# DonghuiZhuo/kube-batch-1

Measured on AMD Instinct MI355X. Metric: pod placements/sec + p50 session latency, 100k nodes × 1M pods, higher is better.
Workload: dtype int64

## Files before the change

kube-batch-1_amd/csrc/engine/engine_dev.h:

```cpp
#pragma once
#include <hip/hip_runtime.h>

#define KBHIP_STAMPS_OFF
#include "../kbhip_batch.h"
#include "../kbhip_engine.h"

namespace kbhip {

constexpr uint64_t kEngWaitTicks = 200000000ull;
constexpr uint64_t kEngArriveTicks = 500000ull;
constexpr uint64_t kEngDescTicks = 400000000ull;

__device__ __forceinline__ uint64_t eng_now() { return __builtin_amdgcn_s_memrealtime(); }

#define ETL(A, p, ev)                                                                                    \
    do {                                                                                                 \
        if ((A).tl && (threadIdx.x & 63) == 0)                                                           \
            (A).tl[(size_t)((p) % kEngTlSlots) * kEngTlEvents + (ev)] = __builtin_amdgcn_s_memrealtime(); \
    } while (0)

#ifndef KBHIP_POLL_DEPTH
#define KBHIP_POLL_DEPTH 1
#endif
#ifndef KBHIP_POLL_SLEEP
// ... 33 lines not shown
__device__ __forceinline__ T eng_uniform(const T& v) {
    static_assert(sizeof(T) % 4 == 0, "dwords");
    T r;
    const uint32_t* s = (const uint32_t*)&v;
    uint32_t* d = (uint32_t*)&r;
#pragma unroll
    for (int i = 0; i < (int)(sizeof(T) / 4); ++i) d[i] = (uint32_t)__builtin_amdgcn_readfirstlane((int)s[i]);
    return r;
}

__device__ __forceinline__ TaskClass eng_class(const uint32_t* w) {
    return eng_uniform(*(const TaskClass*)(w + kEngDescClass));
}
__device__ __forceinline__ TaskClass eng_class_x(uint32_t x) {
    TaskClass c;
    uint32_t* d = (uint32_t*)&c;
#pragma unroll
    for (int i = 0; i < (int)(sizeof(TaskClass) / 4); ++i)
        d[i] = (uint32_t)__builtin_amdgcn_readlane((int)x, kEngDescClass + i);
    return c;
}

struct EngDesc {
    uint32_t op, cls, m, gang, ent32, min_avail, ready, epoch, slot;
    int32_t kbase, kshift, kidxmax;
};
__device__ __forceinline__ EngDesc eng_decode(const uint32_t* w) {
    EngDesc d;
    d.cls = w[kDwCls];
    d.m = w[kDwFlags] & 0xff;
    d.gang = (w[kDwFlags] >> 8) & 1;
    d.ent32 = (w[kDwFlags] >> 9) & 1;
    d.op = (w[kDwFlags] >> 12) & 0xf;
    d.min_avail = w[kDwMinAvail];
    d.ready = w[kDwReady];
    d.epoch = w[kDwEpochSlot] & 0xffff;
    d.slot = w[kDwEpochSlot] >> 16;
    d.kbase = (int32_t)w[kDwKbase];
    d.kshift = (int32_t)w[kDwKshift];
    d.kidxmax = (int32_t)w[kDwKidxmax];
    return d;
}
__device__ __forceinline__ PopArgs eng_args(const EngDesc& d) {
    PopArgs a{};
    a.cls = (int32_t)d.cls;
    a.n_tasks = (int32_t)d.m;
    a.gang_mode = (int32_t)d.gang;
    a.min_avail = (int32_t)d.min_avail;
    a.ready_count = (int32_t)d.ready;
    a.epoch = d.epoch;
    a.placement = 2;
    a.kbase = d.kbase;
    a.kshift = d.kshift;
    a.kidxmax = d.kidxmax;
    a.ent32 = (int32_t)d.ent32;
    a.fit_set = 0;
    return a;
}

__device__ __forceinline__ bool eng_wait_desc(EngCtl* ctl, uint32_t p, uint32_t* w) {
    const int lane = threadIdx.x & 63;
    const uint64_t* src = &ctl->desc[p % kEngRing][lane];
    EngWait wt(ctl, kEngDescTicks);
    for (;;) {
        const uint64_t x = ld_sc1(src);
        if (__ballot((uint32_t)(x >> 32) != p) == 0) {
            w[lane] = (uint32_t)x;
            return true;
        }
        if (!wt.tick(kEngErrDesc)) return false;
    }
}

__device__ __forceinline__ bool eng_wait_done(EngCtl* ctl, uint32_t want) {
    EngWait wt(ctl, kEngWaitTicks);
    for (;;) {
        const uint32_t v = (uint32_t)__builtin_amdgcn_readfirstlane((int)ld_sc1(&ctl->done));
        if ((int32_t)(v - want) >= 0) return true;
        if (!wt.tick()) return false;
    }
}

constexpr int kPollDepth = KBHIP_POLL_DEPTH;
__device__ __forceinline__ bool eng_poll_tag(EngCtl* ctl, const uint64_t* w, uint32_t q, uint64_t limit) {
    uint64_t v[kPollDepth];
#pragma unroll
    for (int i = 0; i < kPollDepth; ++i) {
        v[i] = ld_sc1(w);
        eng_pause();
    }
    EngWait wt(ctl, limit);
    for (;;) {
#pragma unroll
        for (int i = 0; i < kPollDepth; ++i) {
            if ((uint32_t)__builtin_amdgcn_readfirstlane((int)(uint32_t)(v[i] >> 32)) == q) return true;
            v[i] = ld_sc1(w);
            if (!wt.tick()) return false;
        }
    }
}

__device__ __forceinline__ bool eng_poll_tags(EngCtl* ctl, const uint64_t* w, uint32_t q, uint64_t limit) {
    uint64_t v[kPollDepth];
#pragma unroll
    for (int i = 0; i < kPollDepth; ++i) {
        v[i] = w ? ld_sc1(w) : ((uint64_t)q << 32);
        eng_pause();
    }
    bool seen = false;
    EngWait wt(ctl, limit);
    for (;;) {
#pragma unroll
        for (int i = 0; i < kPollDepth; ++i) {
            seen = seen || (uint32_t)(v[i] >> 32) == q;
            if (__ballot(!seen) == 0) return true;
            v[i] = (w && !seen) ? ld_sc1(w) : ((uint64_t)q << 32);
            if (!wt.tick()) return false;
        }
    }
}

__device__ __forceinline__ bool eng_wait_cands(EngCtl* ctl, uint32_t q, int* node, int copy) {
    const int lane = threadIdx.x & 63;
    const uint64_t* src = &ctl->cands[q % kEngSlots][copy % kEngCandCopies][lane];
    if (!eng_poll_tag(ctl, &ctl->cands[q % kEngSlots][copy % kEngCandCopies][0], q, kEngWaitTicks)) return false;
    EngWait wt(ctl, kEngWaitTicks);
    for (;;) {
        const uint64_t x = ld_sc1(src);
        if (__ballot((uint32_t)(x >> 32) != q) == 0) {
            *node = (int)(uint32_t)x;
            return true;
        }
        if (!wt.tick()) return false;
    }
}

template <typename T>
__device__ __forceinline__ void block_merge128_all(T (*w0)[64], T (*w1)[64], T a0, T a1, int wave, int lane) {
    w0[wave][lane] = a0;
    w1[wave][lane] = a1;
    __syncthreads();
#pragma unroll
    for (int s = kPopThreads / 128; s >= 1; s >>= 1) {
        if (wave < s) {
            T x0 = w0[wave][lane], x1 = w1[wave][lane];
            wave_merge128_desc(x0, x1, w0[wave + s][lane], w1[wave + s][lane]);
            w0[wave][lane] = x0;
            w1[wave][lane] = x1;
        }
        __syncthreads();
    }
}

__device__ __forceinline__ void block_merge256_all(uint32_t (*wl)[kPopThreads / 64][64], const uint32_t* a, int wave,
                                                   int lane) {
#pragma unroll
    for (int k = 0; k < 4; ++k) wl[k][wave][lane] = a[k];
    __syncthreads();
#pragma unroll
    for (int s = kPopThreads / 128; s >= 1; s >>= 1) {
        if (wave < s) {
            uint32_t x[4], y[4];
#pragma unroll
            for (int k = 0; k < 4; ++k) { x[k] = wl[k][wave][lane]; y[k] = wl[k][wave + s][lane]; }
            wave_merge256_desc(x, y);
#pragma unroll
            for (int k = 0; k < 4; ++k) wl[k][wave][lane] = x[k];
        }
        __syncthreads();
    }
}

__device__ __forceinline__ uint32_t wave_sum_u32(uint32_t x) {
    x += __shfl_xor(x, 1, 64);
    x += __shfl_xor(x, 2, 64);
    x += __shfl_xor(x, 4, 64);
    x += __shfl_xor(x, 8, 64);
    x += __shfl_xor(x, 16, 64);
// ... 114 lines not shown
```

kube-batch-1_amd/csrc/engine/engine_owner.h:

```cpp
#pragma once
#include <hip/hip_runtime.h>

#define KBHIP_STAMPS_OFF
#include "../kbhip_batch.h"
#include "../kbhip_engine.h"
#include "engine_dev.h"

namespace kbhip {

__device__ __forceinline__ uint32_t own_val(uint64_t k64, int32_t kbase) {
    if (!k64) return 0;
    return ((uint32_t)(key_score(k64) - kbase + 1) << 1) | (uint32_t)(k64 & 1);
}
__device__ __forceinline__ uint32_t own_key(uint32_t v, int g, const EngArgs& A) {
    return ((v >> 1) << A.kshift) | ((uint32_t)(A.kidxmax - g) << 1) | (v & 1);
}
__device__ __forceinline__ void own_count(EngOwnerLds& L, int n, uint32_t v, uint32_t d) {
    if (!v) return;
    const uint32_t lv = v >> 1;
    atomicAdd(&L.lvl[lv], d);
    atomicAdd(&L.seg[lv >> 1][n / kOwnSeg], d << (16 * (lv & 1)));
}
__device__ __forceinline__ uint32_t own_segcnt(const EngOwnerLds& L, int lv, int sg) {
    return (L.seg[lv >> 1][sg] >> (16 * (lv & 1))) & 0xffffu;
// ... 308 lines not shown
        const uint32_t nk = min(L.nkeys, (uint32_t)kOwnPre);
        uint32_t r[4];
#pragma unroll
        for (int k = 0; k < 4; ++k) r[k] = (uint32_t)(64 * k + lane) < nk ? L.keys[64 * k + lane] : 0u;
#pragma unroll
        for (int k = 0; k < 4; ++k) r[k] = wave_sort_desc(r[k]);
        uint32_t n[4];
        {
            const uint32_t rv = reverse_lanes(r[1]);
            m[0] = bitonic_clean_desc(r[0] > rv ? r[0] : rv);
            m[1] = bitonic_clean_desc(r[0] > rv ? rv : r[0]);
        }
        {
            const uint32_t rv = reverse_lanes(r[3]);
            n[0] = bitonic_clean_desc(r[2] > rv ? r[2] : rv);
            n[1] = bitonic_clean_desc(r[2] > rv ? rv : r[2]);
        }
        m[2] = m[3] = n[2] = n[3] = 0u;
        wave_merge256_desc(m, n);
        ETL(A, p, 12);
    }
    __syncthreads();
    if (xs3 >= 0) { L.hkey[xs3] = -1; L.hval[xs3] = -1; }
    if ((int32_t)(p - 3 - A.first) >= 0 && (int32_t)(*ap - (p - 3)) < 0) {
        if (wave == 0) {
            EngWait wt(ctl, kEngWaitTicks);
            while ((int32_t)((uint32_t)__builtin_amdgcn_readfirstlane((int)ld_sc1(&ctl->done)) - (p - 3)) < 0)
                if (!wt.tick()) { if (lane == 0) L.ok = 0; break; }
        }
        __syncthreads();
        if (!L.ok) return false;
        if (!own_apply(cf, nc, t, c, A, L, fbh, kbase, p - 3, 1, false)) return false;
        *ap = p - 3;
        own_drain();
        if (threadIdx.x == 0) st_sc1(&ctl->own_ap[blockIdx.x], *ap);
    }
    __syncthreads();
    if (wave == 0) {
        const uint32_t v = x3 >= 0 ? (uint32_t)L.sv[x3] : 0u;
        const uint32_t k3 = wave_sort_desc(v ? own_key(v, x3 + nc.base, A) : 0u);
        const uint32_t b[4] = {k3, 0u, 0u, 0u};
        wave_merge256_desc(m, b);
        __builtin_amdgcn_s_waitcnt(0xc07f);
        __builtin_amdgcn_wave_barrier();
#pragma unroll
        for (int k = 0; k < 4; ++k) L.keys[64 * k + lane] = m[k];
    }
    int x2 = -1;
    if (wave == 1) {
        if ((int32_t)(p - 2 - A.first) >= 0) ok = own_log_node(ctl, p - 2, &x2);
        if (!ok && lane == 0) L.ok = 0;
        ETL(A, p, 11);
    }
    bool xf2 = false;
    int xs2 = -1;
    if (x2 >= 0) xs2 = own_hinsert(L, x2, &xf2);
    const uint32_t xfb2 = xf2 ? ld_sc1(&fbh[x2]) : 0u;
    __syncthreads();
    bool keep = false;
    uint64_t km = 0;
    if (wave < 4) {
        const uint32_t k = L.keys[64 * wave + lane];
        keep = k && own_hfind(L, key_node(k, a) - nc.base) < 0;
        km = __ballot(keep);
        if (lane == 0) L.wcnt[wave] = (uint32_t)__popcll(km);
    }
    __syncthreads();
    if (wave < 4) {
        uint32_t base = 0;
        for (int w = 0; w < wave; ++w) base += L.wcnt[w];
        const uint32_t tot = L.wcnt[0] + L.wcnt[1] + L.wcnt[2] + L.wcnt[3];
        const uint32_t pos = base + __builtin_amdgcn_mbcnt_hi((uint32_t)(km >> 32), __builtin_amdgcn_mbcnt_lo((uint32_t)km, 0));
        if (keep && pos < (uint32_t)kEngPkgN) L.slot_entry[pos] = 64 * wave + lane;
        if (wave < 2 && (uint32_t)(64 * wave + lane) >= tot) L.slot_entry[64 * wave + lane] = -1;
    }
    __syncthreads();
    EngPkg* pk = A.pkg + (p % kEngSlots);
    const uint64_t tag = (uint64_t)p << 32;
    if (wave < 2) {
        const int e = 64 * wave + lane;
        const int src = L.slot_entry[e];
        const uint32_t k = src >= 0 ? L.keys[src] : 0u;
        const int n = k ? key_node(k, a) - nc.base : -1;
        uint32_t v[kEngPkgFields];
#pragma unroll
        for (int f = 0; f < kEngPkgFields; ++f) v[f] = 0;
        v[kPkKey] = k;
        if (n >= 0) {
            const Row r = load_row_sc1(nc, n);
            const uint8_t fl = nc.flags[n];
            const int32_t na = cf.score_mult ? na_weight(c, t, nc, n) : 0;
            const uint64_t pw[4] = {0, 0, 0, 0};
            const uint32_t* rw = (const uint32_t*)&r;
#pragma unroll
            for (int f = 0; f < (int)(sizeof(Row) / 4); ++f) v[kPkRow + f] = rw[f];
            v[kPkFlags] = fl;
            v[kPkNa] = (uint32_t)na;
            v[kPkS1] = (uint32_t)depth1_score(cf, nc, t, c, r, pw, n, na, key64_of(k, a));
        }
#pragma unroll
        for (int f = 0; f < kEngPkgFields; ++f) st_sc1(&pk->w[f][e], tag | v[f]);
        asm volatile("s_waitcnt vmcnt(0)" ::: "memory");
        if (wave == 0) ETL(A, p, 13);
    }
    if (wave == 1) {
#pragma unroll
        for (int b = 0; b < 4; ++b) {
            const int kx = __popcll(__ballot(xf2 && ((xfb2 >> b) & 1u)));
            if (lane == 0 && kx) atomicAdd((uint32_t*)&L.xfit[b], (uint32_t)kx);
        }
    }
    __syncthreads();
    if (threadIdx.x == 0) st_sc1(&A.ctl->pkg_ready[p % kEngSlots][0], tag | 1u);
    if (wave == 2 && L.ok) {
        int n1 = -1;
        if ((int32_t)(p - 1 - A.first) >= 0) ok = own_log_node(ctl, p - 1, &n1);
        const bool in = ok && n1 >= 0 && own_hfind(L, n1) < 0;
        const uint32_t fb1 = in ? ld_sc1(&fbh[n1]) : 0u;
        uint32_t cnt = 0;
#pragma unroll
        for (int b = 0; b < 4; ++b) {
            const uint32_t k = (uint32_t)__popcll(__ballot(in && ((fb1 >> b) & 1u)));
            if (lane == b) cnt = L.fit[b] - (uint32_t)L.xfit[b] - k;
        }
        if (ok && lane < 4) st_sc1(&A.blists[(size_t)(p % kEngSlots) * kEngListWords + 128 + lane], tag | cnt);
        if (!ok && lane == 0) L.ok = 0;
        ETL(A, p, 18);
    }
    __syncthreads();
    if (xs2 >= 0) { L.hkey[xs2] = -1; L.hval[xs2] = -1; }
    return L.ok != 0;
}

__device__ __forceinline__ void eng_owner(const Conf& cf, const NodeCols& nc, const DevTables& t, const EngArgs& A,
                                          EngOwnerLds& L, int o) {
    const int lane = threadIdx.x & 63, wave = threadIdx.x >> 6;
    EngCtl* ctl = A.ctl;
    const int cls = A.own_cls[o];
    const int32_t kbase = A.own_kbase[o];
    const TaskClass& c = t.classes[cls];
    uint8_t* fbh = A.own_fb + (size_t)o * nc.npad;
    const int N = nc.n;
    for (int i = threadIdx.x; i < kOwnLv / 2 * kOwnSegs; i += kPopThreads) (&L.seg[0][0])[i] = 0;
    for (int i = threadIdx.x; i < kOwnHash; i += kPopThreads) { L.hkey[i] = -1; L.hval[i] = -1; }
    for (int i = threadIdx.x; i < kOwnMaxN / kOwnSub; i += kPopThreads) L.smax[i] = 0;
    for (int i = threadIdx.x; i < kOwnLv; i += kPopThreads) L.lvl[i] = 0;
    if (threadIdx.x < 4) L.fit[threadIdx.x] = 0;
    if (threadIdx.x == 0) L.ok = 1;
    __syncthreads();
    const int nend = ((N + kOwnSeg - 1) / kOwnSeg) * kOwnSeg;
    for (int n0 = 0; n0 < nend; n0 += 2 * kPopThreads) {
        uint32_t v[2] = {0, 0}, fb[2] = {0, 0};
        uint64_t k[2] = {0, 0};
#pragma unroll
        for (int u = 0; u < 2; ++u) {
            const int n = n0 + u * kPopThreads + (int)threadIdx.x;
            if (n < N) k[u] = eng_eval(cf, c, t, nc, n, &fb[u]);
        }
#pragma unroll
        for (int u = 0; u < 2; ++u) {
            const int n = n0 + u * kPopThreads + (int)threadIdx.x;
            v[u] = own_val(k[u], kbase);
            if (n < nend) L.sv[n] = (uint8_t)v[u];
            {
                uint32_t mx = v[u] >> 1;
#pragma unroll
                for (int dd = 1; dd < 64; dd <<= 1) mx = max(mx, (uint32_t)__shfl_xor((int)mx, dd, 64));
                if (lane == 0 && n < nend) atomicMax(&L.smax[n / kOwnSub], mx);
            }
            if (n < N) fbh[n] = (uint8_t)fb[u];
            fit_block_add(L.fit, fb[u]);
            uint64_t act = __ballot(v[u] != 0);
            while (act) {
                const int l0 = __builtin_ctzll(act);
                const uint32_t lv = (uint32_t)__shfl((int)v[u], l0, 64) >> 1;
                const uint64_t m = __ballot(v[u] != 0 && (v[u] >> 1) == lv);
                if (lane == l0) {
                    atomicAdd(&L.lvl[lv], (uint32_t)__popcll(m));
                    atomicAdd(&L.seg[lv >> 1][n / kOwnSeg], (uint32_t)__popcll(m) << (16 * (lv & 1)));
                }
                act &= ~m;
            }
        }
    }
    asm volatile("s_waitcnt vmcnt(0)" ::: "memory");
    __syncthreads();
    uint32_t ap = A.first - 1;
    uint32_t dp = A.first;
    uint64_t t0 = 0;
    int seen = -1;
    for (;;) {
        if (wave == 0) {
            bool ok = own_scan_desc(A, L, cls, dp);
            if (!ok && lane == 0) L.ok = 0;
        } else if (wave == 1) {
            const uint32_t dn = ld_sc1(&ctl->done);
// ... 58 lines not shown
```

kube-batch-1_amd/csrc/engine/engine_placer.h:

```cpp
#pragma once
#include <hip/hip_runtime.h>

#define KBHIP_STAMPS_OFF
#include "../kbhip_batch.h"
#include "../kbhip_engine.h"
#include "engine_dev.h"

namespace kbhip {

static_assert(sizeof(Row) == 4 * (kPkFlags - kPkRow), "the package carries a Row as 28 32-bit words");
static_assert(kEngDescClass + sizeof(TaskClass) / 4 <= kEngDescWords, "a descriptor carries its class");

template <typename ET>
__device__ __forceinline__ Row eng_row_after(const TaskClass& c, const PlaceDec<ET>& D, const Row& base) {
    const int cc = D.cc > 0 ? D.cc : 0;
    const int na = cc < D.ap_l ? cc : D.ap_l;
    return apply_commits(base, c, na, cc - na);
}
template <typename ET>
__device__ __forceinline__ void eng_fit_vals(const Conf& cf, const NodeCols& nc, const DevTables& t,
                                             const TaskClass& c, const PopArgs& a, const PlaceDec<ET>& D,
                                             const Row& base, const int32_t* fit_in, uint32_t fit_raw, uint64_t* g0,
                                             uint64_t* g1) {
    uint32_t fb_base = 0, fb_post = 0;
// ... 262 lines not shown
            L.fe[0][lane] = k.e;
            L.ffb[0][lane] = (uint8_t)k.fb;
            L.fkind[0][lane] = (uint8_t)k.kind;
            L.fna[0][lane] = k.na;
            if (k.kind == 2) L.fs1p[0][lane] = k.s1p;
            ETL(A, q - 1, 34);
            L.e[0][lane] = wave_sort_desc(node >= 0 ? k.e : 0u);
            L.fbp[0][lane] = node >= 0 ? (uint8_t)k.fb : (uint8_t)0;
            __builtin_amdgcn_s_waitcnt(0xc07f);
            if (lane == 0) __hip_atomic_store(&L.sort_seq[0], (int)q, __ATOMIC_RELAXED, __HIP_MEMORY_SCOPE_WORKGROUP);
            ETL(A, q - 1, 35);
        } else {
            int32_t s1 = INT32_MIN;
            if (node >= 0) s1 = front_s1a(cf, nc, t, c, node, L.rc.row[src]);
            if (!front_wait(L, &L.rows_seq, (int)(q - 1))) return;
            const int m = L.ccm[lane];
            if (m == 1 && node >= 0 && !own_ring) {
                if (!front_wait(L, &L.v1_seq[1], (int)q)) return;
                s1 = L.v1s1a[lane];
            }
            const bool slow = node >= 0 && (m > 1 || own_ring);
            if (__ballot(slow) != 0 && slow) s1 = front_s1a(cf, nc, t, c, node, L.rc.row[sl]);
            if (node >= 0) L.fs1a[0][lane] = s1;
        }
        return;
    }
    if (role == 0) ETL(A, q - 1, 32 + 4 * set);
    const int node = L.xn[ring][lane];
    if (role == 0) {
        FrontKey k{0u, 0u, 0u, 0, INT32_MIN};
        if (node >= 0) k = front_key(cf, nc, t, c, a, node, L.rc.row[sl], L.flags[sl]);
        ETL(A, q - 1, 33 + 4 * set);
        L.fe[set][lane] = k.e;
        L.ffb[set][lane] = (uint8_t)k.fb;
        L.fkind[set][lane] = (uint8_t)k.kind;
        L.fna[set][lane] = k.na;
        if (k.kind == 2) L.fs1p[set][lane] = k.s1p;
        bool hashed = false;
        for (int i = 0; i < 4096 && !hashed; ++i) {
            hashed = __hip_atomic_load(&L.hash_seq, __ATOMIC_RELAXED, __HIP_MEMORY_SCOPE_WORKGROUP) == (int)q;
            if (!hashed) __builtin_amdgcn_s_sleep(1);
        }
        ETL(A, q - 1, 34 + 4 * set);
        if (hashed) {
            const bool use = node >= 0 && (set == 1 ? L.x2use[lane] : L.x3use[lane]);
            L.e[set][lane] = wave_sort_desc(use ? k.e : 0u);
            L.fbp[set][lane] = use ? (uint8_t)k.fb : (uint8_t)0;
            __builtin_amdgcn_s_waitcnt(0xc07f);
            if (lane == 0) __hip_atomic_store(&L.sort_seq[set], (int)q, __ATOMIC_RELAXED, __HIP_MEMORY_SCOPE_WORKGROUP);
            ETL(A, q - 1, 35 + 4 * set);
        }
    } else if (node >= 0) {
        L.fs1a[set][lane] = front_s1a(cf, nc, t, c, node, L.rc.row[sl]);
    }
}

__device__ __forceinline__ void eng_front_v1(const Conf& cf, const NodeCols& nc, const DevTables& t,
                                             EngPlacerLds& L, uint32_t q, uint32_t dw, int role) {
    const int lane = eng_lane();
    uint32_t w[8];
#pragma unroll
    for (int i = 0; i < 8; ++i) w[i] = (uint32_t)__builtin_amdgcn_readlane((int)dw, i);
    const PopArgs a = eng_args(eng_decode(w));
    const TaskClass c = eng_class_x(dw);
    if (!front_wait(L, &L.xn_seq, (int)(q - 1))) return;
    const TaskClass& cp = *(const TaskClass*)&L.desc[(q - 1) % 2][kEngDescClass];
    const int ring = (int)((q + 3) % 4);
    const int node = L.xn[ring][lane];
    if (node >= 0) {
        const int src = L.srcslot[lane];
        const Row r = apply_commits(L.rc.row[src], cp, 1, 0);
        if (role == 0) {
            const FrontKey k = front_key(cf, nc, t, c, a, node, r, L.flags[src]);
            L.v1e[lane] = k.e; L.v1fb[lane] = (uint8_t)k.fb; L.v1kind[lane] = (uint8_t)k.kind; L.v1s1p[lane] = k.s1p;
        } else {
            L.v1s1a[lane] = front_s1a(cf, nc, t, c, node, r);
        }
    }
    __builtin_amdgcn_s_waitcnt(0xc07f);
    if (lane == 0) __hip_atomic_store(&L.v1_seq[role], (int)q, __ATOMIC_RELAXED, __HIP_MEMORY_SCOPE_WORKGROUP);
}

template <int K>
__device__ __forceinline__ void front_pkg_store(EngPlacerLds& L, const uint64_t (&v)[16], int base, uint32_t q,
                                                int lane) {
    EngRowCache& rc = L.rc;
#pragma unroll
    for (int i = 0; i < 16; ++i) {
        constexpr int kF0 = 8 * K;
        const int f = kF0 + (i >> 1), e = lane + 64 * (i & 1), sl = base + e;
        const uint32_t x = (uint32_t)v[i];
        if (f == kPkKey) L.pkey[q % 2][e] = x;
        else if (f < kPkFlags) ((uint32_t*)&rc.row[sl])[f - kPkRow] = x;
        else if (f == kPkFlags) L.flags[sl] = (uint8_t)x;
        else if (f == kPkNa) rc.na[sl] = (int32_t)x;
        else rc.s1[sl] = (int32_t)x;
    }
}

template <bool LIST>
__device__ __forceinline__ void eng_front(const Conf& cf, const NodeCols& nc, const DevTables& t, const EngArgs& A,
                                          EngPlacerLds& L, uint32_t q, int wave) {
    const int lane = threadIdx.x & 63;
    EngCtl* ctl = A.ctl;
    EngRowCache& rc = L.rc;
    if (wave == 0) return;
    const int k = wave == 3 ? 0 : wave == 4 ? 1 : wave - 4;
    const EngPkg* pk = A.pkg + (q % kEngSlots);
    uint64_t v[16];
    uint32_t dw;
    if (__hip_atomic_load(&L.ndesc_seq, __ATOMIC_RELAXED, __HIP_MEMORY_SCOPE_WORKGROUP) == (int)q) {
        dw = L.ndesc[lane];
    } else {
        const uint64_t* src = &ctl->desc[q % kEngRing][lane];
        EngWait wt(ctl, kEngDescTicks);
        uint64_t x = 0;
        for (;;) {
            x = ld_sc1(src);
            if (__ballot((uint32_t)(x >> 32) != q) == 0) break;
            if (!wt.tick(kEngErrDesc)) {
                if (wave == 3 && lane == 0) L.ok = 0;
                return;
            }
        }
        dw = (uint32_t)x;
    }
    if (wave == 3) L.desc[q % 2][lane] = dw;
    if (((uint32_t)__builtin_amdgcn_readlane((int)dw, kDwFlags) >> 12 & 0xf) != kEngOpPop) return;
    if (wave == 2) {
        const int r1 = (int)((q + 3) % 4), r2 = (int)((q + 2) % 4), r3 = (int)((q + 1) % 4);
        while (__hip_atomic_load(&L.xn_seq, __ATOMIC_RELAXED, __HIP_MEMORY_SCOPE_WORKGROUP) != (int)(q - 1)) {
            if (!__hip_atomic_load(&L.ok, __ATOMIC_RELAXED, __HIP_MEMORY_SCOPE_WORKGROUP)) return;
            __builtin_amdgcn_s_sleep(1);
        }
        for (int h = lane; h < EngRowCache::kHashN; h += 64) rc.hkey[h] = -1;
        __builtin_amdgcn_s_waitcnt(0xc07f);
        __builtin_amdgcn_wave_barrier();
        const int n1 = L.xn[r1][lane];
        if (n1 >= 0) rc_insert(&rc, n1, 64 * r1 + lane);
        __builtin_amdgcn_s_waitcnt(0xc07f);
        __builtin_amdgcn_wave_barrier();
        const int n2 = L.xn[r2][lane];
        const bool use2 = n2 >= 0 && rc_find(&rc, n2) < 0;
        L.x2use[lane] = use2;
        if (use2) rc_insert(&rc, n2, 64 * r2 + lane);
        if (!LIST) {
            __builtin_amdgcn_s_waitcnt(0xc07f);
            __builtin_amdgcn_wave_barrier();
            const int n3 = L.xn[r3][lane];
            const bool use3 = n3 >= 0 && rc_find(&rc, n3) < 0;
            L.x3use[lane] = use3;
            if (use3) rc_insert(&rc, n3, 64 * r3 + lane);
        }
        __builtin_amdgcn_s_waitcnt(0xc07f);
        if (lane == 0) __hip_atomic_store(&L.hash_seq, (int)q, __ATOMIC_RELAXED, __HIP_MEMORY_SCOPE_WORKGROUP);
        ETL(A, q - 1, 63);
        eng_front_eval<LIST>(cf, nc, t, A, L, q, dw, 0, 1);
        return;
    }
    if constexpr (LIST) {
        if (wave == 1) { eng_front_eval<LIST>(cf, nc, t, A, L, q, dw, 0, 0); return; }
        if (wave == 5) { eng_front_v1(cf, nc, t, L, q, dw, 1); return; }
        if (wave == 3) eng_front_eval<LIST>(cf, nc, t, A, L, q, dw, 1, 1);
        else if (wave == 6) eng_front_eval<LIST>(cf, nc, t, A, L, q, dw, 1, 0);
        else if (wave == 7) eng_front_v1(cf, nc, t, L, q, dw, 0);
    } else {
        if (wave == 1) { eng_front_eval<LIST>(cf, nc, t, A, L, q, dw, 0, 0); return; }
        if (wave == 5) { eng_front_eval<LIST>(cf, nc, t, A, L, q, dw, 1, 1); return; }
        if (wave == 3) eng_front_eval<LIST>(cf, nc, t, A, L, q, dw, 2, 1);
        else if (wave == 6) eng_front_eval<LIST>(cf, nc, t, A, L, q, dw, 1, 0);
        else if (wave == 7) eng_front_eval<LIST>(cf, nc, t, A, L, q, dw, 2, 0);
    }
    ETL(A, q - 1, 56 + k);
    bool got = false;
    if (!eng_poll_tag(ctl, &ctl->pkg_ready[q % kEngSlots][0], q, kEngWaitTicks)) {
        if (k == 0 && lane == 0) L.ok = 0;
        return;
    }
#pragma unroll
    for (int i = 0; i < 16; ++i) v[i] = ld_sc1(&pk->w[8 * k + (i >> 1)][lane + 64 * (i & 1)]);
    EngWait wt(ctl, kEngWaitTicks);
    for (;;) {
        bool miss = false;
#pragma unroll
        for (int i = 0; i < 16; ++i) miss |= (uint32_t)(v[i] >> 32) != q;
        if (__ballot(miss) == 0) { got = true; break; }
#pragma unroll
        for (int i = 0; i < 16; ++i)
            if ((uint32_t)(v[i] >> 32) != q) v[i] = ld_sc1(&pk->w[8 * k + (i >> 1)][lane + 64 * (i & 1)]);
        if (!wt.tick()) break;
    }
    if (got) {
        ETL(A, q - 1, 48 + k);
        const int base = kEngStage + kEngPkgN * (int)(q % 2);
        switch (k) {
            case 0: front_pkg_store<0>(L, v, base, q, lane); break;
            case 1: front_pkg_store<1>(L, v, base, q, lane); break;
            case 2: front_pkg_store<2>(L, v, base, q, lane); break;
            default: front_pkg_store<3>(L, v, base, q, lane); break;
        }
        ETL(A, q - 1, 52 + k);
        if (k == 0) {
            for (int w = 0; w < 4; ++w) { rc.pw[base + lane][w] = 0; rc.pw[base + 64 + lane][w] = 0; }
            bool hashed = false;
            for (int i = 0; i < 4096 && !hashed; ++i) {
                hashed = __hip_atomic_load(&L.hash_seq, __ATOMIC_RELAXED, __HIP_MEMORY_SCOPE_WORKGROUP) == (int)q;
                if (!hashed) __builtin_amdgcn_s_sleep(1);
            }
            ETL(A, q - 1, 62);
            if (hashed) {
                uint32_t w8[8];
#pragma unroll
                for (int i = 0; i < 8; ++i) w8[i] = (uint32_t)__builtin_amdgcn_readlane((int)dw, i);
                eng_drop_stale(L, eng_args(eng_decode(w8)), q);
                __builtin_amdgcn_s_waitcnt(0xc07f);
                if (lane == 0) __hip_atomic_store(&L.drop_seq, (int)q, __ATOMIC_RELAXED, __HIP_MEMORY_SCOPE_WORKGROUP);
                ETL(A, q - 1, 60);
                bool both = false;
                for (int i = 0; i < 4096 && !both; ++i) {
                    both = __hip_atomic_load(&L.sort_seq[1], __ATOMIC_RELAXED, __HIP_MEMORY_SCOPE_WORKGROUP) == (int)q &&
                           (LIST ||
                            __hip_atomic_load(&L.sort_seq[2], __ATOMIC_RELAXED, __HIP_MEMORY_SCOPE_WORKGROUP) == (int)q);
                    if (!both) __builtin_amdgcn_s_sleep(1);
                }
                if (both) {
                    uint32_t top = wave_merge_desc(L.s64[lane], L.e[1][lane]);
                    L.pre64[lane] = LIST ? top : wave_merge_desc(top, L.e[2][lane]);
                    __builtin_amdgcn_s_waitcnt(0xc07f);
                    if (lane == 0) __hip_atomic_store(&L.pre_seq, (int)q, __ATOMIC_RELAXED, __HIP_MEMORY_SCOPE_WORKGROUP);
                    ETL(A, q - 1, 61);
                }
            }
        }
    } else if (k == 0 && lane == 0) {
        L.ok = 0;
    }
}

template <bool LIST>
__device__ __forceinline__ void eng_placer(const Conf& cf, const NodeCols& nc, const DevTables& t, const EngArgs& A,
                                           EngPlacerLds& L) {
    const int lane = threadIdx.x & 63, wave = threadIdx.x >> 6;
    EngCtl* ctl = A.ctl;
    EngRowCache& rc = L.rc;
    for (int i = threadIdx.x; i < 4 * 64; i += kPopThreads) L.xn[i >> 6][i & 63] = -1;
    if (threadIdx.x == 0) {
        L.ok = 1; L.gran_seq = 0; L.ndesc_seq = 0; L.rows_seq = (int)A.first - 1;
        L.hash_seq = L.drop_seq = (int)A.first - 1;
        L.xn_seq = (int)A.first - 1;
        L.v1_seq[0] = L.v1_seq[1] = L.pre_seq = (int)A.first - 1;
        L.sort_seq[0] = L.sort_seq[1] = L.sort_seq[2] = (int)A.first - 1;
        L.apmin = A.first - 1;
    }
    __syncthreads();
    eng_front<LIST>(cf, nc, t, A, L, A.first, wave);
    uint32_t pend = 0;
    for (uint32_t p = A.first;; ++p) {
        const int r1 = (int)((p + 3) % 4), r2 = (int)((p + 2) % 4), r3 = (int)((p + 1) % 4), r0 = (int)(p % 4);
        __syncthreads();
        if (!L.ok) return;
        const EngDesc d = eng_decode(L.desc[p % 2]);
        if (d.op != kEngOpPop) {
            if (wave == 0) eng_publish_done(ctl, &pend);
            return;
        }
        const PopArgs a = eng_args(d);
        const TaskClass& c = *(const TaskClass*)&L.desc[p % 2][kEngDescClass];
        if (wave == 0) {
            ETL(A, p, 0);
            if (lane == 0 && A.tl) A.tl[(size_t)(p % kEngTlSlots) * kEngTlEvents + 31] = p;
        }
        if (wave == 0) {
            if (__hip_atomic_load(&L.drop_seq, __ATOMIC_RELAXED, __HIP_MEMORY_SCOPE_WORKGROUP) != (int)p)
                eng_drop_stale(L, a, p);
            ETL(A, p, 1);
        } else if (wave == 4) {
// ... 174 lines not shown
```

kube-batch-1_amd/csrc/engine/engine_sweep.h:

```cpp
#pragma once
#include <hip/hip_runtime.h>

#define KBHIP_STAMPS_OFF
#include "../kbhip_batch.h"
#include "../kbhip_engine.h"
#include "engine_dev.h"

namespace kbhip {

__device__ __forceinline__ void eng_fit_drop(EngWorkerLds& L, int set, int node, int lo, int cnt) {
    const int lane = threadIdx.x & 63;
    const int o = node - lo;
    const bool own = node >= 0 && o >= 0 && o < cnt;
    uint32_t fb = 0;
    if (own) {
        fb = L.fb[set][o];
        L.fb[set][o] = 0;
    }
#pragma unroll
    for (int q = 0; q < 4; ++q) {
        const int k = __popcll(__ballot((fb >> q) & 1u));
        if (lane == q && k) atomicSub(&L.fitb[set][q], (uint32_t)k);
    }
    __builtin_amdgcn_s_waitcnt(0xc07f);
// ... 248 lines not shown
        if (!L.ok) return;
        if (eng_decode(L.desc).op != kEngOpPop) return;
        const uint64_t* src0 = A.blists + (size_t)(p % kEngSlots) * A.nw * kEngListWords;
        uint32_t a0 = 0, a1 = 0;
        bool ok = eng_merge_lists(ctl, src0, g, A.ng, cg, p, &a0, &a1);
        if (!ok) L.ok = 0;
        if (g == 0 && wave == 0) ETL(A, p, 25);
        block_merge128_all(L.wl, L.wl2, a0, a1, wave, lane);
        if (!L.ok) return;
        if (wave == 0) {
            uint64_t* dst = A.glists + ((size_t)(p % kEngSlots) * A.ng + g) * kEngListWords;
            st_sc1(&dst[lane], ((uint64_t)p << 32) | L.wl[0][lane]);
            st_sc1(&dst[64 + lane], ((uint64_t)p << 32) | L.wl2[0][lane]);
            if (g == 0) ETL(A, p, 26);
            if (cpub + 1 < p) {
                eng_group_counts(A, g, cg, p - 1, true, &ok);
                cpub = p - 1;
            }
            if (!ok && lane == 0) L.ok = 0;
            if (g == 0) ETL(A, p, 27);
        }
    }
}

__device__ __forceinline__ void eng_final(const Conf& cf, const NodeCols& nc, const DevTables& t, const EngArgs& A,
                          EngMergerLds& L) {
    const int lane = threadIdx.x & 63, wave = threadIdx.x >> 6;
    EngCtl* ctl = A.ctl;
    if (threadIdx.x == 0) L.ok = 1;
    for (uint32_t p = A.first;; ++p) {
        __syncthreads();
        if (!L.ok) return;
        if (wave == 0) {
            const bool ok = eng_wait_desc(ctl, p, L.desc);
            if (lane == 0) L.ok = ok;
            ETL(A, p, 20);
        }
        __syncthreads();
        if (!L.ok) return;
        const EngDesc d = eng_decode(L.desc);
        if (d.op != kEngOpPop) return;
        const PopArgs a = eng_args(d);
        const TaskClass c = eng_class(L.desc);
        uint32_t a0 = 0, a1 = 0;
        bool ok = true;
        if (A.ng == 0) {
            ok = eng_merge_lists(ctl, A.blists + (size_t)(p % kEngSlots) * A.nw * kEngListWords, 0, 1, A.nw, p, &a0,
                                 &a1);
        } else if (wave < A.ng) {
            constexpr int kFinalDepth = 4;
            const uint64_t* s = A.glists + ((size_t)(p % kEngSlots) * A.ng + wave) * kEngListWords;
            uint64_t v0[kFinalDepth], v1[kFinalDepth];
#pragma unroll
            for (int i = 0; i < kFinalDepth; ++i) {
                v0[i] = ld_sc1(&s[lane]);
                v1[i] = ld_sc1(&s[64 + lane]);
                __builtin_amdgcn_s_sleep(2);
            }
            bool got = false;
            EngWait wt(ctl, kEngWaitTicks);
            while (!got) {
#pragma unroll
                for (int i = 0; i < kFinalDepth; ++i) {
                    if (__ballot((uint32_t)(v0[i] >> 32) != p || (uint32_t)(v1[i] >> 32) != p) == 0) {
                        a0 = (uint32_t)v0[i];
                        a1 = (uint32_t)v1[i];
                        got = true;
                        break;
                    }
                    v0[i] = ld_sc1(&s[lane]);
                    v1[i] = ld_sc1(&s[64 + lane]);
                    if (!wt.tick()) break;
                }
                if (!got && ld_sc1(&ctl->err) != 0) break;
            }
            ok = got;
        }
        if (!ok) L.ok = 0;
        block_merge128_all(L.wl, L.wl2, a0, a1, wave, lane);
        if (!L.ok) return;
        if (wave == 0) ETL(A, p, 21);
        EngPkg* pk = A.pkg + (p % kEngSlots);
        const uint64_t tag = (uint64_t)p << 32;
        if (wave < 2) {
            const int e = 64 * wave + lane;
            const uint32_t k = wave == 0 ? L.wl[0][lane] : L.wl2[0][lane];
            const int n = k ? key_node(k, a) : -1;
            uint32_t v[kEngPkgFields];
#pragma unroll
            for (int f = 0; f < kEngPkgFields; ++f) v[f] = 0;
            v[kPkKey] = k;
            if (n >= 0) {
                const Row r = load_row_sc1(nc, n);
                const uint8_t fl = nc.flags[n];
                const int32_t na = cf.score_mult ? na_weight(c, t, nc, n) : 0;
                const uint64_t pw[4] = {0, 0, 0, 0};
                const uint32_t* rw = (const uint32_t*)&r;
#pragma unroll
                for (int f = 0; f < (int)(sizeof(Row) / 4); ++f) v[kPkRow + f] = rw[f];
                v[kPkFlags] = fl;
                v[kPkNa] = (uint32_t)na;
                v[kPkS1] = (uint32_t)depth1_score(cf, nc, t, c, r, pw, n, na, key64_of(k, a));
            }
#pragma unroll
            for (int f = 0; f < kEngPkgFields; ++f) st_sc1(&pk->w[f][e], tag | v[f]);
            asm volatile("s_waitcnt vmcnt(0)" ::: "memory");
        }
        if (wave == 0) ETL(A, p, 22);
        __syncthreads();
        if (threadIdx.x == 0) st_sc1(&ctl->pkg_ready[p % kEngSlots][0], tag | 1u);
    }
}

}
```

kube-batch-1_amd/csrc/kbhip_engine.h:

```cpp
#pragma once
#include <stdint.h>

namespace kbhip {

constexpr int kEngRing = 8;
constexpr int kEngHostRing = 16;
constexpr int kEngSlots = 4;
constexpr int kEngMaxGroups = 8;
constexpr int kEngListWords = 136;
constexpr int kEngMaxNpb = 8192;
constexpr int kEngWorkersMax = 512;
#ifndef KBHIP_CAND_COPIES
#define KBHIP_CAND_COPIES 8
#endif
constexpr int kEngCandCopies = KBHIP_CAND_COPIES;

constexpr int kEngPkgN = 128, kEngPkgFields = 32;
enum : int { kPkKey = 0, kPkRow = 1, kPkFlags = 29, kPkNa = 30, kPkS1 = 31 };
struct EngPkg {
    uint64_t w[kEngPkgFields][kEngPkgN];
};

constexpr int kEngDescWords = 64, kEngDescClass = 8;
enum : int { kDwCls = 0, kDwFlags, kDwMinAvail, kDwReady, kDwEpochSlot, kDwKbase, kDwKshift, kDwKidxmax };
enum : uint32_t { kEngOpPop = 0, kEngOpExit = 1 };

constexpr int kEngLog = 64;
constexpr int kEngOwnMax = 256;
constexpr int kOwnSeg = 1792, kOwnSegs = 64, kOwnMaxN = kOwnSeg * kOwnSegs;
static_assert(kOwnSeg % 256 == 0, "a segment is whole scan steps (64 lanes x 4 nodes)");
constexpr int kOwnLv = 128;

struct EngCtl {
    uint32_t done;
    uint32_t pad0[31];
    uint32_t err;
    uint32_t pad1[31];
    uint32_t arrive;
    uint32_t pad2[63];
    uint64_t desc[kEngRing][kEngDescWords];
    uint64_t cands[kEngSlots][kEngCandCopies][64];
    uint64_t pkg_ready[kEngSlots][16];
    uint64_t tlog[kEngLog][64];
    uint64_t tcls[kEngLog];
    uint32_t own_ap[kEngOwnMax];
};
enum : uint32_t { kEngErrWait = 1, kEngErrDesc = 2, kEngErrClass = 3, kEngErrResident = 4 };

struct EngArgs {
    EngCtl* ctl;
    uint64_t* blists;
    uint64_t* glists;
    EngPkg* pkg;
    const uint64_t* hring;
    uint64_t* hexit;
    uint32_t idle_ticks;
    void* out;
    uint32_t first;
    int nw, npb, ng;
    uint64_t* tl;
    int quick;
    int nown;
    const int32_t* own_cls;
    const int32_t* own_kbase;
    uint8_t* own_fb;
    int kshift, kidxmax;
};
constexpr uint32_t kEngIdleTicks = 10000000u;
constexpr int kEngTlSlots = 32768, kEngTlEvents = 64;

}
```

Baseline: 3.037 million.

## Shrink candidate package to untagged 32-bit words with fill count in ready flag

Package words are now 32-bit without per-word epoch tags by default. The producer publishes the valid entry count inside the ready flag, and it only writes rows for real candidates. The consumer polls the flag, reads the count, and loads only the lanes that are filled, skipping the per-word tag re-poll loop. This halves package traffic and drops stores and loads for empty slots. Correctness now rests on the producer's s_waitcnt before the flag store, plus a compiler barrier, to order the data stores ahead of the flag.

```diff
diff --git a/kube-batch-1_amd/csrc/engine/engine_dev.h b/kube-batch-1_amd/csrc/engine/engine_dev.h
--- a/kube-batch-1_amd/csrc/engine/engine_dev.h
+++ b/kube-batch-1_amd/csrc/engine/engine_dev.h
@@ -139,7 +139,8 @@
 }
 
 constexpr int kPollDepth = KBHIP_POLL_DEPTH;
-__device__ __forceinline__ bool eng_poll_tag(EngCtl* ctl, const uint64_t* w, uint32_t q, uint64_t limit) {
+__device__ __forceinline__ bool eng_poll_tag(EngCtl* ctl, const uint64_t* w, uint32_t q, uint64_t limit,
+                                             uint32_t* lo = nullptr) {
     uint64_t v[kPollDepth];
 #pragma unroll
     for (int i = 0; i < kPollDepth; ++i) {
@@ -150,7 +151,10 @@
     for (;;) {
 #pragma unroll
         for (int i = 0; i < kPollDepth; ++i) {
-            if ((uint32_t)__builtin_amdgcn_readfirstlane((int)(uint32_t)(v[i] >> 32)) == q) return true;
+            if ((uint32_t)__builtin_amdgcn_readfirstlane((int)(uint32_t)(v[i] >> 32)) == q) {
+                if (lo) *lo = (uint32_t)__builtin_amdgcn_readfirstlane((int)(uint32_t)v[i]);
+                return true;
+            }
             v[i] = ld_sc1(w);
             if (!wt.tick()) return false;
         }
diff --git a/kube-batch-1_amd/csrc/engine/engine_owner.h b/kube-batch-1_amd/csrc/engine/engine_owner.h
--- a/kube-batch-1_amd/csrc/engine/engine_owner.h
+++ b/kube-batch-1_amd/csrc/engine/engine_owner.h
@@ -414,11 +414,9 @@
         const int src = L.slot_entry[e];
         const uint32_t k = src >= 0 ? L.keys[src] : 0u;
         const int n = k ? key_node(k, a) - nc.base : -1;
-        uint32_t v[kEngPkgFields];
-#pragma unroll
-        for (int f = 0; f < kEngPkgFields; ++f) v[f] = 0;
-        v[kPkKey] = k;
         if (n >= 0) {
+            uint32_t v[kEngPkgFields];
+            v[kPkKey] = k;
             const Row r = load_row_sc1(nc, n);
             const uint8_t fl = nc.flags[n];
             const int32_t na = cf.score_mult ? na_weight(c, t, nc, n) : 0;
@@ -429,9 +427,9 @@
             v[kPkFlags] = fl;
             v[kPkNa] = (uint32_t)na;
             v[kPkS1] = (uint32_t)depth1_score(cf, nc, t, c, r, pw, n, na, key64_of(k, a));
-        }
-#pragma unroll
-        for (int f = 0; f < kEngPkgFields; ++f) st_sc1(&pk->w[f][e], tag | v[f]);
+#pragma unroll
+            for (int f = 0; f < kEngPkgFields; ++f) st_sc1(&pk->w[f][e], eng_pkg_word(tag, v[f]));
+        }
         asm volatile("s_waitcnt vmcnt(0)" ::: "memory");
         if (wave == 0) ETL(A, p, 13);
     }
@@ -443,7 +441,10 @@
         }
     }
     __syncthreads();
-    if (threadIdx.x == 0) st_sc1(&A.ctl->pkg_ready[p % kEngSlots][0], tag | 1u);
+    if (threadIdx.x == 0) {
+        const uint32_t tot = L.wcnt[0] + L.wcnt[1] + L.wcnt[2] + L.wcnt[3];
+        st_sc1(&A.ctl->pkg_ready[p % kEngSlots][0], tag | eng_pkg_flag(tot < (uint32_t)kEngPkgN ? tot : (uint32_t)kEngPkgN));
+    }
     if (wave == 2 && L.ok) {
         int n1 = -1;
         if ((int32_t)(p - 1 - A.first) >= 0) ok = own_log_node(ctl, p - 1, &n1);
diff --git a/kube-batch-1_amd/csrc/engine/engine_placer.h b/kube-batch-1_amd/csrc/engine/engine_placer.h
--- a/kube-batch-1_amd/csrc/engine/engine_placer.h
+++ b/kube-batch-1_amd/csrc/engine/engine_placer.h
@@ -368,7 +368,7 @@
 }
 
 template <int K>
-__device__ __forceinline__ void front_pkg_store(EngPlacerLds& L, const uint64_t (&v)[16], int base, uint32_t q,
+__device__ __forceinline__ void front_pkg_store(EngPlacerLds& L, const EngPkgWord (&v)[16], int base, uint32_t q,
                                                 int lane) {
     EngRowCache& rc = L.rc;
 #pragma unroll
@@ -384,6 +384,15 @@
     }
 }
 
+__device__ __forceinline__ bool eng_poll_pkg(EngCtl* ctl, const uint64_t* w, uint32_t q, uint64_t limit, uint32_t* n) {
+    uint32_t lo = 0;
+    if (!eng_poll_tag(ctl, w, q, limit, &lo)) return false;
+    const uint32_t fill = eng_pkg_fill(lo);
+    *n = fill < (uint32_t)kEngPkgN ? fill : (uint32_t)kEngPkgN;
+    asm volatile("" ::: "memory");
+    return true;
+}
+
 template <bool LIST>
 __device__ __forceinline__ void eng_front(const Conf& cf, const NodeCols& nc, const DevTables& t, const EngArgs& A,
                                           EngPlacerLds& L, uint32_t q, int wave) {
@@ -393,7 +402,7 @@
     if (wave == 0) return;
     const int k = wave == 3 ? 0 : wave == 4 ? 1 : wave - 4;
     const EngPkg* pk = A.pkg + (q % kEngSlots);
-    uint64_t v[16];
+    EngPkgWord v[16];
     uint32_t dw;
     if (__hip_atomic_load(&L.ndesc_seq, __ATOMIC_RELAXED, __HIP_MEMORY_SCOPE_WORKGROUP) == (int)q) {
         dw = L.ndesc[lane];
@@ -458,26 +467,44 @@
         else if (wave == 7) eng_front_eval<LIST>(cf, nc, t, A, L, q, dw, 2, 0);
     }
     ETL(A, q - 1, 56 + k);
-    bool got = false;
-    if (!eng_poll_tag(ctl, &ctl->pkg_ready[q % kEngSlots][0], q, kEngWaitTicks)) {
+    uint32_t n = 0;
+    if (!eng_poll_pkg(ctl, &ctl->pkg_ready[q % kEngSlots][0], q, kEngWaitTicks, &n)) {
         if (k == 0 && lane == 0) L.ok = 0;
         return;
     }
 #pragma unroll
-    for (int i = 0; i < 16; ++i) v[i] = ld_sc1(&pk->w[8 * k + (i >> 1)][lane + 64 * (i & 1)]);
+    for (int i = 0; i < 16; ++i) v[i] = 0;
+    const bool in0 = lane < (int)n, in1 = 64 + lane < (int)n;
+    if (n > 64) {
+#pragma unroll
+        for (int i = 0; i < 16; i += 2) v[i] = ld_sc1(&pk->w[8 * k + (i >> 1)][lane]);
+        if (in1) {
+#pragma unroll
+            for (int i = 1; i < 16; i += 2) v[i] = ld_sc1(&pk->w[8 * k + (i >> 1)][64 + lane]);
+        }
+    } else if (in0) {
+#pragma unroll
+        for (int i = 0; i < 16; i += 2) v[i] = ld_sc1(&pk->w[8 * k + (i >> 1)][lane]);
+    }
+    bool got = true;
+#if KBHIP_PKG_TAGGED
+    got = false;
     EngWait wt(ctl, kEngWaitTicks);
     for (;;) {
         bool miss = false;
 #pragma unroll
-        for (int i = 0; i < 16; ++i) miss |= (uint32_t)(v[i] >> 32) != q;
+        for (int i = 0; i < 16; ++i) miss |= ((i & 1) ? in1 : in0) && (uint32_t)(v[i] >> 32) != q;
         if (__ballot(miss) == 0) { got = true; break; }
 #pragma unroll
         for (int i = 0; i < 16; ++i)
-            if ((uint32_t)(v[i] >> 32) != q) v[i] = ld_sc1(&pk->w[8 * k + (i >> 1)][lane + 64 * (i & 1)]);
+            if (((i & 1) ? in1 : in0) && (uint32_t)(v[i] >> 32) != q)
+                v[i] = ld_sc1(&pk->w[8 * k + (i >> 1)][lane + 64 * (i & 1)]);
         if (!wt.tick()) break;
     }
+#endif
     if (got) {
-        ETL(A, q - 1, 48 + k);
+        if (A.tl && lane == 0)
+            A.tl[(size_t)((q - 1) % kEngTlSlots) * kEngTlEvents + 48 + k] = eng_now() | ((uint64_t)n << 56);
         const int base = kEngStage + kEngPkgN * (int)(q % 2);
         switch (k) {
             case 0: front_pkg_store<0>(L, v, base, q, lane); break;
diff --git a/kube-batch-1_amd/csrc/engine/engine_sweep.h b/kube-batch-1_amd/csrc/engine/engine_sweep.h
--- a/kube-batch-1_amd/csrc/engine/engine_sweep.h
+++ b/kube-batch-1_amd/csrc/engine/engine_sweep.h
@@ -354,15 +354,15 @@
         if (wave == 0) ETL(A, p, 21);
         EngPkg* pk = A.pkg + (p % kEngSlots);
         const uint64_t tag = (uint64_t)p << 32;
+        uint32_t fill = 0;
+        if (wave == 0) fill = (uint32_t)(__popcll(__ballot(L.wl[0][lane] != 0)) + __popcll(__ballot(L.wl2[0][lane] != 0)));
         if (wave < 2) {
             const int e = 64 * wave + lane;
             const uint32_t k = wave == 0 ? L.wl[0][lane] : L.wl2[0][lane];
             const int n = k ? key_node(k, a) : -1;
-            uint32_t v[kEngPkgFields];
-#pragma unroll
-            for (int f = 0; f < kEngPkgFields; ++f) v[f] = 0;
-            v[kPkKey] = k;
             if (n >= 0) {
+                uint32_t v[kEngPkgFields];
+                v[kPkKey] = k;
                 const Row r = load_row_sc1(nc, n);
                 const uint8_t fl = nc.flags[n];
                 const int32_t na = cf.score_mult ? na_weight(c, t, nc, n) : 0;
@@ -373,15 +373,15 @@
                 v[kPkFlags] = fl;
                 v[kPkNa] = (uint32_t)na;
                 v[kPkS1] = (uint32_t)depth1_score(cf, nc, t, c, r, pw, n, na, key64_of(k, a));
-            }
-#pragma unroll
-            for (int f = 0; f < kEngPkgFields; ++f) st_sc1(&pk->w[f][e], tag | v[f]);
+#pragma unroll
+                for (int f = 0; f < kEngPkgFields; ++f) st_sc1(&pk->w[f][e], eng_pkg_word(tag, v[f]));
+            }
             asm volatile("s_waitcnt vmcnt(0)" ::: "memory");
         }
         if (wave == 0) ETL(A, p, 22);
         __syncthreads();
-        if (threadIdx.x == 0) st_sc1(&ctl->pkg_ready[p % kEngSlots][0], tag | 1u);
-    }
-}
-
-}
+        if (threadIdx.x == 0) st_sc1(&ctl->pkg_ready[p % kEngSlots][0], tag | eng_pkg_flag(fill));
+    }
+}
+
+}
diff --git a/kube-batch-1_amd/csrc/kbhip_engine.h b/kube-batch-1_amd/csrc/kbhip_engine.h
--- a/kube-batch-1_amd/csrc/kbhip_engine.h
+++ b/kube-batch-1_amd/csrc/kbhip_engine.h
@@ -15,11 +15,27 @@
 #endif
 constexpr int kEngCandCopies = KBHIP_CAND_COPIES;
 
+#ifndef KBHIP_PKG_TAGGED
+#define KBHIP_PKG_TAGGED 0
+#endif
 constexpr int kEngPkgN = 128, kEngPkgFields = 32;
 enum : int { kPkKey = 0, kPkRow = 1, kPkFlags = 29, kPkNa = 30, kPkS1 = 31 };
+#if KBHIP_PKG_TAGGED
+using EngPkgWord = uint64_t;
+#else
+using EngPkgWord = uint32_t;
+#endif
 struct EngPkg {
-    uint64_t w[kEngPkgFields][kEngPkgN];
+    EngPkgWord w[kEngPkgFields][kEngPkgN];
 };
+static_assert(sizeof(EngPkg) == sizeof(EngPkgWord) * kEngPkgFields * kEngPkgN && sizeof(EngPkg) % 256 == 0,
+              "a package is its words, whole lines (the host sizes the slots by sizeof(EngPkg))");
+constexpr EngPkgWord eng_pkg_word(uint64_t tag, uint32_t v) {
+    return KBHIP_PKG_TAGGED ? (EngPkgWord)(tag | v) : (EngPkgWord)v;
+}
+constexpr uint32_t kEngPkgReady = 1u << 31;
+constexpr uint32_t eng_pkg_flag(uint32_t n) { return kEngPkgReady | n; }
+constexpr uint32_t eng_pkg_fill(uint32_t flag_lo) { return flag_lo & 0xffu; }
 
 constexpr int kEngDescWords = 64, kEngDescClass = 8;
 enum : int { kDwCls = 0, kDwFlags, kDwMinAvail, kDwReady, kDwEpochSlot, kDwKbase, kDwKshift, kDwKidxmax };
diff --git a/profiles/engine_pkg_tl.py b/profiles/engine_pkg_tl.py
--- /dev/null
+++ b/profiles/engine_pkg_tl.py
@@ -0,0 +1,97 @@
+#!/usr/bin/env python3
+import argparse
+import json
+import os
+import sys
+
+import numpy as np
+
+ROOT = os.path.dirname(os.path.dirname(os.path.abspath(__file__)))
+sys.path.insert(0, os.path.join(ROOT, "kube-batch-1_amd"))
+import kbgen
+import kbhip
+
+SLOTS, EV = 32768, 64
+TMASK = (1 << 56) - 1
+
+
+def main():
+    ap = argparse.ArgumentParser()
+    ap.add_argument("--nodes", type=int, default=100_000)
+    ap.add_argument("--pending", type=int, default=800_000)
+    ap.add_argument("--lists", type=int, default=0)
+    ap.add_argument("--out", default="")
+    ap.add_argument("--npz", default="")
+    ap.add_argument("--fills", default="", help="npz of another run: its fill counts by pop")
+    a = ap.parse_args()
+    path = f"/tmp/kbhip_bench/c4_{a.nodes}_{a.pending}_{kbgen.BASE_SEED + 4}.kbs"
+    if not os.path.exists(path):
+        os.makedirs(os.path.dirname(path), exist_ok=True)
+        kbgen.gen_c4(path, n_nodes=a.nodes, n_pending=a.pending)
+    buf = open(path, "rb").read()
+    with kbhip.Session(buf) as s:
+        s.allocate()
+    with kbhip.Session(buf) as s:
+        s.set_option("engine_lists", a.lists)
+        s.set_option("engine_timeline", 1)
+        s.allocate()
+        st = s.stats()
+        raw = np.zeros(SLOTS * EV, np.uint64)
+        n = kbhip.lib().kbhip_debug_table(s._h, b"engine_tl", raw.ctypes.data, raw.nbytes)
+        assert n == raw.nbytes
+    t = raw.reshape(SLOTS, EV)
+    fill = (t[:, 48] >> np.uint64(56)).astype(np.int64)
+    t = (t & np.uint64(TMASK)).astype(np.int64)
+    t[:, 31] = raw.reshape(SLOTS, EV)[:, 31].astype(np.int64)
+    order = np.argsort(t[:, 31])
+    t, fill = t[order], fill[order]
+    keep = (t[:, 31] > 100) & np.all(t[:, [0, 5, 48, 52, 60, 61, 62, 63]] > 0, axis=1)
+    t, fill = t[keep], fill[keep]
+    pops = t[:, 31]
+    if a.fills:
+        z = np.load(a.fills)
+        by_pop = dict(zip(z["pops"].tolist(), z["fill"].tolist()))
+        fill = np.array([by_pop.get(int(p), -1) for p in pops])
+    us = lambda x: round(float(np.median(x)) / 100.0, 3) if len(x) else None
+    nxt = np.diff(pops) == 1
+    per = {}
+    rel = lambda ev: t[:, ev] - t[:, 5]
+    for k, w in enumerate((3, 4, 6, 7)):
+        per[f"wave {w}: evaluation done ({56 + k})"] = us(rel(56 + k))
+        per[f"wave {w}: block {k} in registers ({48 + k})"] = us(rel(48 + k))
+        per[f"wave {w}: block {k} in LDS ({52 + k})"] = us(rel(52 + k))
+    per["hash done (63)"] = us(rel(63))
+    per["drop done (60)"] = us(rel(60))
+    per["front's end: merged with sets 1, 2 (61)"] = us(rel(61))
+    flag = (t[1:, 22] - t[:-1, 5])[nxt & (t[1:, 22] > 0)]
+    per["package flagged (22 of pop q)"] = us(flag)
+    ok = nxt & (t[1:, 22] > 0)
+    per["flagged -> keys in registers"] = us((t[:-1, 48] - t[1:, 22])[ok & (t[:-1, 48] > t[1:, 22])])
+    per["share of pops whose flag precedes the wave's poll"] = round(float(np.mean((t[1:, 22] < t[:-1, 56])[ok])), 3)
+    per["eval done -> keys in registers (poll + load)"] = us(t[:, 48] - t[:, 56])
+    per["keys in registers -> in LDS"] = us(t[:, 52] - t[:, 48])
+    per["keys in LDS -> drop done (incl. the wait for the hash)"] = us(t[:, 60] - t[:, 52])
+    per["hash seen (62) -> drop done (60)"] = us(t[:, 60] - t[:, 62])
+    per["drop done -> front's end"] = us(t[:, 61] - t[:, 60])
+    period = np.diff(t[:, 0])
+    per["period"] = us(period[nxt])
+    f0 = fill[:-1]
+    per["period, pops with n = 0"] = us(period[nxt & (f0 == 0)])
+    per["period, pops with n > 0"] = us(period[nxt & (f0 > 0)])
+    per["period, pops with n = 128"] = us(period[nxt & (f0 == 128)])
+    hist = {int(k): int(v) for k, v in zip(*np.unique(np.minimum(fill, 129) // 16 * 16, return_counts=True))}
+    res = {"pops": int(len(t)), "lists": a.lists, "fill_hist_by_16": hist, "pops_n0": int((fill == 0).sum()),
+           "stats": {k: st[k] for k in ("engine_pops", "engine_launches", "engine_workers", "engine_owners",
+                                        "alloc_device_s", "batched_pops", "host_wait_s", "unassigned_pops") if k in st},
+           "median_us": per,
+           "period_mean_us": round(float(period[nxt].mean()) / 100.0, 3)}
+    print(json.dumps(res))
+    if a.out:
+        with open(a.out, "w") as f:
+            json.dump(res, f, indent=1)
+    if a.npz:
+        np.savez_compressed(a.npz, pops=pops + 1, fill=fill)
+
+
+if __name__ == "__main__":
+    main()
```

After: 3.126 million, median of 6. 2.9% higher.
